# researchmm/MM-Diffusion

Hardware: AMD Instinct MI355X
Metric: denoising steps/sec (video+audio pair), 16x64x64 / 25600 (higher is better)
Workload: dtype bf16; 1 GPU; BASELINE configs[1]: Landscape base model (133.68M params), DDPM p_sample, timestep_respacing=250, per-GPU batch 4, 16x3x64x64 video + 1x25600 audio; global_batch=4, parallelism=batch-sharded x1, no in-loop collective, weights=key-seeded synthetic (mm_diffusion.synth), graph_replay=True, batch_lanes=2, finite=True, ranks_seen=1

## Files before the change

### include/mmd.h

```cpp
#ifndef MMD_H
#define MMD_H
#include <stdint.h>
#ifdef __cplusplus
extern "C" {
#endif

#define MMD_F32 0
#define MMD_BF16 1
#define MMD_OK 0
#define MMD_ERR_ARG (-1)
#define MMD_ERR_LAUNCH (-2)
#define MMD_ERR_UNSUPPORTED (-3)

int mmd_version(void);
const char* mmd_last_error(void);
int mmd_debug_install_crash_handler(void);

int mmd_graph_begin(void* stream);
int mmd_graph_end(void* stream, void** exec_out);
int mmd_graph_launch(void* exec, void* stream);
int mmd_graph_destroy(void* exec);
int mmd_stream_create(void** stream_out);
int mmd_stream_sync(void* stream);
int mmd_stream_destroy(void* stream);
int mmd_event_create(void** ev);
int mmd_event_record(void* ev, void* stream);
int mmd_stream_wait_event(void* stream, void* ev);
int mmd_event_elapsed_ms(void* ev_start, void* ev_stop, float* ms);
int mmd_event_destroy(void* ev);

int mmd_temb_fwd(const void* t, int t_kind, int N, int dim, const float* W0, const float* b0, const float* W2,
                 const float* b2, float* out_silu, float* out_raw, void* stream);

int mmd_linear_fwd(const float* x, const float* W, const float* b, float* y, int N, int K, int J, void* stream);

int64_t mmd_gn_workspace_bytes(int dtype, int C, int S, int Tn);
int mmd_gn_stats(int dtype, const void* x, int64_t ld, int C, int S, int Tn, int inner, int64_t outer_stride,
                 int64_t inner_stride, int64_t tstride, const float* gamma, const float* beta, const float* film,
                 int64_t film_ld, float eps, float* a_out, float* b_out, float* mr_out, void* workspace, void* stream);
int mmd_gn_finalize_stats(const float* rec, int64_t rec_ld, int C, int S, int Tn, const float* gamma, const float* beta,
                          const float* film, int64_t film_ld, float eps, float* a_out, float* b_out, float* mr_out, void* stream);
int mmd_gn_apply(int dtype, const void* x, int64_t ldx, void* y, int64_t ldy, int64_t rows, int C, int S, int Tn, int inner,
                 int64_t outer_stride, int64_t inner_stride, int64_t tstride, const float* a, const float* b, int act,
                 void* stream);
int mmd_add_rowbias(int dtype, void* x, int64_t ld, int64_t rows, int C, int64_t rows_per_sample, const float* e,
                    int64_t e_ld, void* stream);
int mmd_colsum_slices(int dtype, const void* dY, int64_t lddy, int S, int64_t Tn, int C, float* out, int64_t ldo, void* stream);

int mmd_conv_gemm(int dtype, const void* A, int64_t lda, const void* W, const float* bias, const void* R, int64_t ldr,
                  void* Y, int64_t ldy, int M, int Cout, int Cin, int ntaps, const int* taps, int D0, int D1, int D2, int tile,
                  void* stream);

int mmd_gn_conv1x1(int dtype, const void* A, int64_t lda, const float* gn_a, const float* gn_b, int act, int S,
                   int64_t rows_per_slice, const void* W, const float* bias, const void* R, int64_t ldr, void* Y, int64_t ldy,
                   int M, int Cout, int Cin, int tile, void* stream);

int mmd_gn_small(int dtype, const void* x, int64_t ldx, void* y, int64_t ldy, int C, int S, int Tn, int inner, int64_t outer_stride,
                 int64_t inner_stride, int64_t tstride, const float* gamma, const float* beta, float eps, int act, void* stream);

int mmd_gn_group(int dtype, const void* x, int64_t ldx, void* y, int64_t ldy, int C, int S, int Tn, int inner, int64_t outer_stride,
                 int64_t inner_stride, int64_t tstride, const float* gamma, const float* beta, const float* film, int64_t film_ld,
                 float eps, int act, float* a_out, float* b_out, float* mr_out, void* stream);

int mmd_zero(void* ptr, int64_t bytes, void* stream);

int mmd_conv_gemm_stats(int dtype, const void* A, int64_t lda, const void* W, const float* bias, const void* R, int64_t ldr,
                        void* Y, int64_t ldy, int M, int Cout, int Cin, int ntaps, const int* taps, int D0, int D1, int D2, int tile,
                        float* stats, int64_t stats_ld, void* stream);
int mmd_gn_conv1x1_stats(int dtype, const void* A, int64_t lda, const float* gn_a, const float* gn_b, int act, int S,
                         int64_t rows_per_slice, const void* W, const float* bias, const void* R, int64_t ldr, void* Y, int64_t ldy,
                         int M, int Cout, int Cin, int tile, float* stats, int64_t stats_ld, void* stream);

int mmd_gn_conv1x1_skip(int dtype, const void* h, int64_t ldh, const float* gn_a, const float* gn_b, int act, int S,
                        int64_t rows_per_slice, const void* W_out, const float* bias_out, const void* x, int64_t ldx, int K2,
                        const void* W_skip, const float* bias_skip, void* Y, int64_t ldy, int M, int Cout, int K1, float* stats,
                        int64_t stats_ld, void* stream);

int mmd_gn_conv_gemm(int dtype, const void* A, int64_t lda, const float* gn_a, const float* gn_b, int act, int S,
                     int64_t rows_per_slice, const void* W, const float* bias, const void* R, int64_t ldr, void* Y, int64_t ldy,
                     int M, int Cout, int Cin, int ntaps, const int* taps, int D0, int D1, int D2, int tile, void* stream);

int64_t mmd_vconv2d1d_weight_bytes(int Cin);
int mmd_vconv2d1d_pack(const void* Ws, const void* Wt, void* out, int Cin, int Cout, void* stream);
int mmd_vconv2d1d(const void* X, int64_t ldx, const float* gn_a, const float* gn_b, int act, int S, int64_t rows_per_slice,
                  const void* Wf, const float* bias_s, const float* bias_t, void* Y, int64_t ldy, int N, int F, int H, int W,
                  int Cin, int Cout, float* stats, int64_t stats_ld, void* stream);

int64_t mmd_tattn_weight_bytes(int C, int with_pre);
int mmd_tattn_pack(const void* Wpre, const void* Wqkv, const void* Wproj, void* out, int C, void* stream);
int mmd_tattn_block(const void* X, int64_t ldx, const void* A, int64_t lda, void* MID, int64_t ldm, const void* Wf,
                    const float* bias_pre, const float* bias_qkv, const float* bias_proj, const float* gamma, const float* beta,
                    float eps, void* Y, int64_t ldy, int N, int F, int HW, int C, int heads, float* stats, int64_t stats_ld,
                    void* stream);

int64_t mmd_tconv_weight_bytes(int Cin, int Cout);
int mmd_tconv_pack(const void* W, void* out, int Cin, int Cout, void* stream);
int mmd_tconv(const void* X, int64_t ldx, const void* Wf, const float* bias, void* Y, int64_t ldy, int N, int F, int HW, int Cin,
              int Cout, float* stats, int64_t stats_ld, void* stream);

int mmd_aconv(const void* X, int64_t ldx, const void* W, const float* bias, const float* ga, const float* gb, int act, void* Y, int64_t ldy,
              int M, int L, int Cin, int Cout, int dil, float* stats, int64_t stats_ld, void* stream);

int mmd_attn_fwd(int dtype, const void* Q, int64_t ldq, int q_off, const void* KV, int64_t ldkv, int k_off, int v_off, void* O,
                 int64_t ldo, int heads, int ch, int nb, int G, int64_t q_rows_per_batch, int q_per_group,
                 int64_t k_rows_per_batch, int k_per_group, int win, const int* shift_dev, int impl, void* stream);
int mmd_attn_small_fwd(int dtype, const void* QKV, int64_t ld, void* O, int64_t ldo, int C, int heads, int S, int Tn, int inner,
                       int64_t outer_stride, int64_t inner_stride, int64_t tstride, void* stream);

int mmd_resample(int dtype, const void* x, int64_t ldx, void* y, int64_t ldy, int C, int NF, int H, int W, int fh, int fw,
                 int mode, float scale, void* stream);
int mmd_resample_stats(const void* x, int64_t ldx, void* y, int64_t ldy, int C, int NF, int H, int W, int fh, int fw, int mode,
                       float* stats, int64_t stats_ld, void* stream);
int mmd_copy2d(const void* x, int64_t ldx_bytes, void* y, int64_t ldy_bytes, int64_t rows, int64_t row_bytes, void* stream);

int mmd_stem_conv(int dtype, const float* x, const float* w, const float* bias, void* y, int64_t ldy, int N, int F, int Cin,
                  int H, int W, int Cout, int ntaps, const int* taps, void* stream);
int mmd_head_conv(int dtype, const void* x, int64_t ldx, const float* w, const float* bias, float* y, int N, int F, int Cin,
                  int H, int W, int Co, int ntaps, const int* taps, void* stream);
int64_t mmd_head_gemm_weight_bytes(int Cin);
int64_t mmd_head_gemm_workspace_bytes(int64_t M, int ntaps, int Co);
int mmd_head_gemm(const void* x, int64_t ldx, int64_t M, int Cin, const float* gn_a, const float* gn_b, int S, int64_t gn_rows, int act,
                  const void* wimg, float* P, int NO, void* stream);
int mmd_head_gather(const float* P, const float* bias, float* y, int N, int F, int H, int W, int Co, int ntaps, const int* taps,
                    void* stream);

int mmd_ddpm_update(const float* x, const float* model_out, const float* noise, float* out, float* x0_out, float* mean_out,
                    float* logvar_out, const float* tables, const int64_t* t, int T, int N, int F, int C, int HW, int flags,
                    void* stream);
int mmd_q_sample(const float* x0, const float* eps, float* out, const float* tab2, const int64_t* t, int T, int N,
// ... 116 lines not shown
```

### mm-diffusion_amd/build.py

```python
#!/usr/bin/env python3
import os
import subprocess
import sys

HERE = os.path.dirname(os.path.abspath(__file__))
SRC = os.path.join(HERE, "csrc")
OUT = os.path.join(HERE, "lib", "libmmd.so")
SOURCES = ["mmd_core.hip", "mmd_gemm.hip", "mmd_vconv.hip", "mmd_tattn.hip", "mmd_tconv.hip", "mmd_aconv.hip", "mmd_norm.hip", "mmd_attn.hip", "mmd_misc.hip", "mmd_edge.hip", "mmd_diffusion.hip", "mmd_bwd.hip", "mmd_attn_bwd.hip", "mmd_attn_bwd_mfma.hip"]
FLAGS = ["--offload-arch=gfx950", "-O3", "-std=c++17", "-fPIC", "-ffp-contract=fast", "-Wno-unused-result", "-Wno-inline-asm"]
FLAGS += os.environ.get("MMD_EXTRA_CXXFLAGS", "").split()
NO_PACKED_F32 = ["-Xclang", "-target-feature", "-Xclang", "-packed-fp32-ops"]
FLAGS += NO_PACKED_F32


def _stale():
    if not os.path.exists(OUT):
        return True
    t = os.path.getmtime(OUT)
    deps = [os.path.join(SRC, f) for f in os.listdir(SRC)] + [os.path.abspath(__file__)]
    return any(os.path.getmtime(d) > t for d in deps)


def _llvm_bin():
    cands = [os.environ.get("LLVM_BIN")]
    hipcc = os.environ.get("HIPCC", "/opt/rocm/bin/hipcc")
    try:
        out = subprocess.run([hipcc, "--print-prog-name=llvm-objdump"], stdout=subprocess.PIPE, stderr=subprocess.DEVNULL, timeout=60).stdout.decode().strip()
        if out and os.path.isabs(out):
            cands.append(os.path.dirname(out))
    except (OSError, subprocess.SubprocessError):
        pass
    cands += [os.path.join(os.path.dirname(os.path.dirname(os.path.realpath(hipcc))), "lib", "llvm", "bin"), "/opt/rocm/lib/llvm/bin"]
    for d in cands:
        if d and os.path.exists(os.path.join(d, "llvm-objdump")):
            return d
    raise RuntimeError("build check: llvm-objdump not found (looked in %s); set LLVM_BIN to the LLVM bin directory of the ROCm toolchain"
                       % ", ".join(str(d) for d in cands if d))


def _code_objects(path, td):
    lib = os.path.join(td, os.path.basename(path))
    os.symlink(os.path.abspath(path), lib)
    subprocess.check_call([os.path.join(_llvm_bin(), "llvm-objdump"), "--offloading", lib], cwd=td, stdout=subprocess.DEVNULL, stderr=subprocess.DEVNULL)
    cos = [f for f in os.listdir(td) if f.startswith(os.path.basename(path) + ".") and f.endswith("gfx950")]
    return [os.path.join(td, f) for f in sorted(cos, key=lambda f: (len(f), f))]


def _check_no_packed_f32(path):
    import re
    import tempfile
    llvm = _llvm_bin()
    with tempfile.TemporaryDirectory() as td:
        cos = _code_objects(path, td)
        if len(cos) < len(SOURCES) - 1:
            raise RuntimeError("build check: expected >= %d gfx950 code objects in %s, found %d" % (len(SOURCES) - 1, path, len(cos)))
        asm = ""
        for f in cos:
            asm += subprocess.run([os.path.join(llvm, "llvm-objdump"), "-d", "--mcpu=gfx950", f],
                                  stdout=subprocess.PIPE, stderr=subprocess.DEVNULL, check=True).stdout.decode(errors="replace")
    n_mfma = len(re.findall(r"\bv_mfma_", asm))
    bad = re.findall(r"\bv_pk_(?:add|mul|fma)_f32\b", asm)
# ... 56 lines not shown
```

### mm-diffusion_amd/mm_diffusion/_hip.py

```python
import ctypes as C
import gc
import os

import torch

_HERE = os.path.dirname(os.path.abspath(__file__))
LIB_PATH = os.environ.get("MMD_LIB") or os.path.join(os.path.dirname(_HERE), "lib", "libmmd.so")

F32, BF16 = 0, 1
_lib = None

i32, i64, f32, vp = C.c_int, C.c_int64, C.c_float, C.c_void_p


_PROTOS = {
    "mmd_version": (C.c_int, []),
    "mmd_last_error": (C.c_char_p, []),
    "mmd_debug_install_crash_handler": (i32, []),
    "mmd_graph_begin": (i32, [vp]),
    "mmd_graph_end": (i32, [vp, C.POINTER(vp)]),
    "mmd_graph_launch": (i32, [vp, vp]),
    "mmd_graph_destroy": (i32, [vp]),
    "mmd_stream_create": (i32, [C.POINTER(vp)]),
    "mmd_stream_sync": (i32, [vp]),
    "mmd_stream_destroy": (i32, [vp]),
    "mmd_event_create": (i32, [C.POINTER(vp)]),
    "mmd_event_record": (i32, [vp, vp]),
    "mmd_stream_wait_event": (i32, [vp, vp]),
    "mmd_event_elapsed_ms": (i32, [vp, vp, C.POINTER(f32)]),
    "mmd_event_destroy": (i32, [vp]),
    "mmd_temb_fwd": (i32, [vp, i32, i32, i32, vp, vp, vp, vp, vp, vp, vp]),
    "mmd_linear_fwd": (i32, [vp, vp, vp, vp, i32, i32, i32, vp]),
    "mmd_gn_workspace_bytes": (i64, [i32, i32, i32, i32]),
    "mmd_gn_stats": (i32, [i32, vp, i64, i32, i32, i32, i32, i64, i64, i64, vp, vp, vp, i64, f32, vp, vp, vp, vp, vp]),
    "mmd_gn_small": (i32, [i32, vp, i64, vp, i64, i32, i32, i32, i32, i64, i64, i64, vp, vp, f32, i32, vp]),
    "mmd_gn_group": (i32, [i32, vp, i64, vp, i64, i32, i32, i32, i32, i64, i64, i64, vp, vp, vp, i64, f32, i32, vp, vp, vp, vp]),
    "mmd_gn_apply": (i32, [i32, vp, i64, vp, i64, i64, i32, i32, i32, i32, i64, i64, i64, vp, vp, i32, vp]),
    "mmd_add_rowbias": (i32, [i32, vp, i64, i64, i32, i64, vp, i64, vp]),
    "mmd_colsum_slices": (i32, [i32, vp, i64, i32, i64, i32, vp, i64, vp]),
    "mmd_conv_gemm": (i32, [i32, vp, i64, vp, vp, vp, i64, vp, i64, i32, i32, i32, i32, C.POINTER(i32), i32, i32, i32, i32, vp]),
    "mmd_gn_conv1x1": (i32, [i32, vp, i64, vp, vp, i32, i32, i64, vp, vp, vp, i64, vp, i64, i32, i32, i32, i32, vp]),
    "mmd_conv_gemm_stats": (i32, [i32, vp, i64, vp, vp, vp, i64, vp, i64, i32, i32, i32, i32, C.POINTER(i32), i32, i32, i32, i32, vp, i64, vp]),
    "mmd_gn_conv1x1_stats": (i32, [i32, vp, i64, vp, vp, i32, i32, i64, vp, vp, vp, i64, vp, i64, i32, i32, i32, i32, vp, i64, vp]),
    "mmd_gn_conv1x1_skip": (i32, [i32, vp, i64, vp, vp, i32, i32, i64, vp, vp, vp, i64, i32, vp, vp, vp, i64, i32, i32, i32, vp, i64, vp]),
    "mmd_gn_conv_gemm": (i32, [i32, vp, i64, vp, vp, i32, i32, i64, vp, vp, vp, i64, vp, i64, i32, i32, i32, i32, C.POINTER(i32), i32, i32, i32, i32, vp]),
    "mmd_tconv_weight_bytes": (i64, [i32, i32]),
    "mmd_tconv_pack": (i32, [vp, vp, i32, i32, vp]),
    "mmd_tconv": (i32, [vp, i64, vp, vp, vp, i64, i32, i32, i32, i32, i32, vp, i64, vp]),
    "mmd_aconv": (i32, [vp, i64, vp, vp, vp, vp, i32, vp, i64, i32, i32, i32, i32, i32, vp, i64, vp]),
    "mmd_tattn_weight_bytes": (i64, [i32, i32]),
    "mmd_tattn_pack": (i32, [vp, vp, vp, vp, i32, vp]),
    "mmd_tattn_block": (i32, [vp, i64, vp, i64, vp, i64, vp, vp, vp, vp, vp, vp, f32, vp, i64, i32, i32, i32, i32, i32, vp, i64, vp]),
    "mmd_vconv2d1d_weight_bytes": (i64, [i32]),
    "mmd_vconv2d1d_pack": (i32, [vp, vp, vp, i32, i32, vp]),
    "mmd_vconv2d1d": (i32, [vp, i64, vp, vp, i32, i32, i64, vp, vp, vp, vp, i64, i32, i32, i32, i32, i32, i32, vp, i64, vp]),
    "mmd_zero": (i32, [vp, i64, vp]),
    "mmd_gn_finalize_stats": (i32, [vp, i64, i32, i32, i32, vp, vp, vp, i64, f32, vp, vp, vp, vp]),
    "mmd_attn_fwd": (i32, [i32, vp, i64, i32, vp, i64, i32, i32, vp, i64, i32, i32, i32, i32, i64, i32, i64, i32, i32, vp, i32, vp]),
    "mmd_attn_small_fwd": (i32, [i32, vp, i64, vp, i64, i32, i32, i32, i32, i32, i64, i64, i64, vp]),
    "mmd_resample": (i32, [i32, vp, i64, vp, i64, i32, i32, i32, i32, i32, i32, i32, f32, vp]),
    "mmd_resample_stats": (i32, [vp, i64, vp, i64, i32, i32, i32, i32, i32, i32, i32, vp, i64, vp]),
    "mmd_copy2d": (i32, [vp, i64, vp, i64, i64, i64, vp]),
    "mmd_stem_conv": (i32, [i32, vp, vp, vp, vp, i64, i32, i32, i32, i32, i32, i32, i32, C.POINTER(i32), vp]),
    "mmd_head_conv": (i32, [i32, vp, i64, vp, vp, vp, i32, i32, i32, i32, i32, i32, i32, C.POINTER(i32), vp]),
    "mmd_head_gemm_weight_bytes": (i64, [i32]),
    "mmd_head_gemm_workspace_bytes": (i64, [i64, i32, i32]),
    "mmd_head_gemm": (i32, [vp, i64, i64, i32, vp, vp, i32, i64, i32, vp, vp, i32, vp]),
    "mmd_head_gather": (i32, [vp, vp, vp, i32, i32, i32, i32, i32, i32, C.POINTER(i32), vp]),
    "mmd_ddpm_update": (i32, [vp, vp, vp, vp, vp, vp, vp, vp, vp, i32, i32, i32, i32, i32, i32, vp]),
    "mmd_loss_workspace_bytes": (i64, [i32]),
    "mmd_loss_terms": (i32, [vp, vp, vp, vp, vp, vp, i32, i32, i32, i32, i32, i32, f32, vp, vp, vp, vp]),
    "mmd_conv_wgrad": (i32, [i32, vp, i64, vp, i64, vp, vp, i32, i32, i32, i32, C.POINTER(i32), i32, i32, i32, i32, vp]),
    "mmd_gn_bwd": (i32, [i32, vp, i64, vp, i64, vp, i64, i64, i32, i32, i32, i32, i64, i64, i64, vp, vp, vp, vp, vp, vp, i64, i32, vp, vp, vp, i64, vp, vp]),
    "mmd_gn_bwd_ws0": (i32, [i32, vp, i64, vp, i64, vp, i64, i64, i32, i32, i32, i32, i64, i64, i64, vp, vp, vp, vp, vp, vp, i64, i32, vp, vp, vp, i64, vp, vp]),
    "mmd_attn_bwd": (i32, [i32, vp, i64, i32, vp, i64, i32, i32, vp, i64, vp, i64, vp, i64, i32, vp, i64, i32, i32, vp, vp, i32, i32, i32, i32,
                           i32, i64, i64, i64, i32, i32, i32, i64, i64, i64, i32, i32, i32, vp, vp]),
    "mmd_timestep_embedding": (i32, [vp, i32, i32, i32, vp, vp]),
    "mmd_attn_fwd_lse": (i32, [i32, vp, i64, i32, vp, i64, i32, i32, vp, i64, i32, i32, i32, i32, i64, i32, i64, i32, i32, vp, vp, vp]),
    "mmd_attn_bwd_mfma": (i32, [vp, i64, i32, vp, i64, i32, i32, vp, i64, vp, i64, vp, i64, i32, vp, i64, i32, i32, vp, vp, i32, i32, i32, i32,
                                i64, i32, i64, i32, i32, vp, vp]),
    "mmd_attn_small_bwd": (i32, [i32, vp, i64, vp, i64, vp, i64, i32, i32, i32, i32, i32, i64, i64, i64, vp]),
    "mmd_ddim_update": (i32, [vp, vp, vp, vp, vp, vp, vp, vp, i32, i32, i32, i32, i32, i32, f32, vp]),
    "mmd_lincomb_t": (i32, [vp, vp, vp, vp, vp, vp, vp, i32, i64, vp]),
    "mmd_lincomb": (i32, [vp, f32, vp, f32, vp, f32, vp, i64, vp]),
    "mmd_cast": (i32, [vp, i32, vp, i32, f32, i64, vp]),
    "mmd_ddpm_update_bwd": (i32, [vp, vp, vp, vp, vp, vp, vp, i32, i32, i64, i32, vp]),
    "mmd_abs_quantile": (i32, [vp, i32, i64, f32, vp, vp]),
    "mmd_clamp_scale": (i32, [vp, vp, f32, i32, i64, vp]),
    "mmd_dpm_err": (i32, [vp, vp, vp, f32, f32, i32, i64, vp, vp]),
    "mmd_bilinear_concat": (i32, [vp, vp, vp, i32, i32, i32, i32, i32, i32, vp]),
    "mmd_bilinear_concat_rows": (i32, [i32, vp, vp, vp, i32, i32, i32, i32, i32, i32, i32, vp]),
    "mmd_pack_conv_weights": (i32, [i32, vp, i32, i32, vp]),
    "mmd_pack_blocks": (i32, [i32, i32, i32]),
    "mmd_unpack_conv_grads": (i32, [vp, i32, i32, vp]),
    "mmd_loss_terms_bwd": (i32, [vp, vp, vp, vp, vp, vp, i32, i32, i32, i32, i32, i32, f32, vp, vp, vp, vp]),
    "mmd_silu": (i32, [i32, vp, vp, vp, i64, vp]),
    "mmd_dropout": (i32, [i32, vp, vp, f32, vp, i64, vp]),
# ... 199 lines not shown
```

### mm-diffusion_amd/mm_diffusion/engine.py

```python
import os
from types import SimpleNamespace

import torch

from . import _hip as H
from . import ops
from .ops import Geom


_EMB_ON_AUDIO_STREAM = ops._flag("MMD_EMB_AUX")
_POOL_NOREUSE = os.environ.get("MMD_POOL_NOREUSE") == "1"
_UP_LOWRES = ops._flag("MMD_UP_LOWRES")
_CROSS_SERIAL = ops._flag("MMD_CROSS_SERIAL")
_RESAMPLE_STATS = ops._flag("MMD_RESAMPLE_STATS")
_SKIP_FUSE = ops._flag("MMD_SKIP_FUSE")


class _Pool:

    def __init__(self, device):
        self.device = device
        self.free = []
        self.all = []

    def get(self, nbytes):
        nbytes = (int(nbytes) + 255) // 256 * 256
        best = None
        for i, raw in enumerate(self.free):
            sz = raw.numel()
            if sz >= nbytes and sz <= 2 * nbytes + 65536 and (best is None or sz < self.free[best].numel()):
                best = i
        if best is not None:
            return self.free.pop(best)
        raw = torch.empty(nbytes, dtype=torch.uint8, device=self.device)
        self.all.append(raw)
        return raw

    def put(self, raw):
        if not _POOL_NOREUSE:
            self.free.append(raw)

    def total_bytes(self):
        return sum(r.numel() for r in self.all)


class UNetEngine:
    def __init__(self, model, N, dtype, device):
        if not torch.cuda.is_available():
            raise H.MMDError("no HIP device visible: the MI355X path cannot run (no CPU fallback)")
        H.lib()
        self.model, self.N, self.dtype, self.device = model, N, dtype, torch.device(device)
        self.F, self.Cv_in, self.H0, self.W0 = model.video_size
        self.Ca_in, self.L0 = model.audio_size
        self.mc = model.model_channels
        self.params = {k: v for k, v in model.named_parameters()}
        for k, v in self.params.items():
            if v.device.type != "cuda":
                raise H.MMDError(f"parameter {k} is on {v.device}: move the model to the GPU first (model.to('cuda'))")
        self._sig = self._signature()
        self.pools = [_Pool(self.device), _Pool(self.device)]
        mode = os.environ.get("MMD_GN_EPILOGUE", "1")
        self.rec_enabled = mode == "2" or (mode != "0" and dtype == torch.bfloat16)
        self._recs = {}
        self._gn_small = ops._flag("MMD_GN_SMALL")
        self._vconv_fused = self._tattn_fused = self._tconv = self._aconv = dtype == torch.bfloat16
        self._deferred = []
        H.reap()
        self._aux, self._side = H.Stream(self.device), H.Stream(self.device)
# ... 99 lines not shown
        return self._packed("edge", key, lambda: ops.pack_edge_weight(self.params[key].detach()))

    def _temporal(self, Hh):
        if ops.HALO_CANDIDATE:
            return dict(taps=ops.TAPS_TEMPORAL_D1, dims=(self.N, self.F, Hh * Hh))
        return dict(taps=ops.TAPS_TEMPORAL, dims=(self.F, Hh * Hh, 1))

    def _gn(self, x, prefix, geom, act, film=None, out=None):
        C = x.shape[1]
        if film is None and self._gn_small and ops.gn_small_ok(x, geom):
            y = self._alloc(x.shape[0], C) if out is None else out
            return ops.gn_small(x, self._f32(prefix + ".GroupNorm.weight"), self._f32(prefix + ".GroupNorm.bias"), geom, act=act, out=y)
        if ops.gn_group_ok(x, geom) and self._rec_ready(x, geom) is None:
            y = self._alloc(x.shape[0], C) if out is None else out
            return ops.gn_group(x, self._f32(prefix + ".GroupNorm.weight"), self._f32(prefix + ".GroupNorm.bias"), geom, film=film, out=y, act=act)
        a, b = self._gn_affine(x, prefix, geom, film)
        y = self._alloc(x.shape[0], C) if out is None else out
        ops.gn_apply(x, a, b, geom, act=act, out=y)
        self._release(a, b)
        return y

    def _gn_affine(self, x, prefix, geom, film):
        C = x.shape[1]
        a = self._alloc(geom.S, C, torch.float32)
        b = self._alloc(geom.S, C, torch.float32)
        gamma, beta = self._f32(prefix + ".GroupNorm.weight"), self._f32(prefix + ".GroupNorm.bias")
        rec = self._rec_ready(x, geom)
        if rec is not None:
            ops.gn_finalize_stats(rec, gamma, beta, geom, film=film, a=a, b=b)
        elif ops.gn_group_ok(x, geom):
            ops.gn_group(x, gamma, beta, geom, film=film, a=a, b=b)
        else:
            ws = self._alloc(ops.gn_workspace_bytes(x, geom) // 8, 1, torch.float64)
            ops.gn_stats(x, gamma, beta, geom, film=film, a=a, b=b, ws=ws)
            self._release(ws)
        return a, b

    def _gn_pw(self, x, gn_prefix, geom, act, wkey, bkey, film=None, residual=None, out=None):
        C = x.shape[1]
        Cout = self.params[wkey].shape[0]
        will_emit = True if (out is not None and self._rec_slice(out)[0] is not None) else None
        if not ops.gn_fusable(geom, C, Cout, x, will_emit, act):
            n1 = self._gn(x, gn_prefix, geom, act, film=film)
            y = self._pw(n1, wkey, bkey, residual=residual, out=out)
            self._release(n1)
            return y
        a, b = self._gn_affine(x, gn_prefix, geom, film)
        y = self._alloc(x.shape[0], Cout) if out is None else out
        ops.gn_conv1x1(x, a, b, geom, act, self._gemm_w(wkey), self._f32(bkey), residual=residual, out=y, **self._stats_kw(y))
        self._release(a, b)
        return y

    def _res_tail(self, s, h, xs, geom, film, make_out):
        if s.cin != s.cout and _SKIP_FUSE and ops.skip_fusable(h, xs, s.cout, geom):
            dest = make_out()
            will_emit = True if self._rec_slice(dest)[0] is not None else None
            if ops.skip_fusable(h, xs, s.cout, geom, will_emit, dest):
                a, b = self._gn_affine(h, s.out_norm, geom, film)
                (wo, bo), (wk, bk) = self._wb(s.out_conv), self._wb(s.skip)
                ops.gn_conv1x1_skip(h, a, b, geom, True, self._gemm_w(wo), self._f32(bo), xs, self._gemm_w(wk), self._f32(bk), out=dest,
                                    stats=self._stats_for(dest))
                self._release(a, b)
                return dest
            sk = self._pw(xs, *self._wb(s.skip))
        else:
            sk = self._pw(xs, *self._wb(s.skip)) if s.cin != s.cout else xs
            dest = make_out()
        self._gn_pw(h, s.out_norm, geom, True, *self._wb(s.out_conv), film=film, residual=sk, out=dest)
        if sk is not xs:
            self._release(sk)
        return dest

    def _pw(self, x, wkey, bkey, residual=None, out=None):
        y = self._alloc(x.shape[0], self.params[wkey].shape[0]) if out is None else out
        return ops.conv_gemm(x, self._gemm_w(wkey), self._f32(bkey), residual=residual, out=y, **self._stats_kw(y))

    def _self_attn(self, x, prefix, kind, Hh, out, pre=None, no_proj=False):
        N, F, C = self.N, self.F, x.shape[1]
        heads = self.model.num_heads
        ch = C // heads
        rows = x.shape[0]
        if kind == "spatial":
            geom = Geom.spatial(N, F, Hh * Hh)
        elif kind == "temporal":
            geom = Geom.temporal(N, F, Hh * Hh)
        else:
            geom = Geom.per_sample(N, rows // N)
        if kind == "temporal" and self._tattn_fused and ops.tattn_fused_ok(x, heads, N, F, Hh * Hh):
            pk = None
            if pre is not None:
                att, sp = pre
                mid = self._alloc(rows, C)
                pk = (att, self._f32(sp + ".proj_out.bias"), mid)
            wf = self._packed("tattn_pre" if pre is not None else "tattn", prefix, lambda: ops.tattn_pack(
                self._gemm_w(prefix + ".qkv.weight"), self._gemm_w(prefix + ".proj_out.weight"),
                wpre=self._gemm_w(pre[1] + ".proj_out.weight") if pre is not None else None))
            ops.tattn_block(x, wf, self._f32(prefix + ".qkv.bias"), self._f32(prefix + ".proj_out.bias"),
                            self._f32(prefix + ".norm.GroupNorm.weight"), self._f32(prefix + ".norm.GroupNorm.bias"), heads, N, F, Hh * Hh,
                            out=out, stats=self._stats_for(out, perm_unit=rows // N), pre=pk)
            if pk is not None:
                self._release(pk[2])
            return out
        qkv = self._gn_pw(x, prefix + ".norm", geom, False, prefix + ".qkv.weight", prefix + ".qkv.bias")
        att = self._alloc(rows, C)
        if kind == "temporal":
            if F > 32:
                raise H.MMDError(f"temporal attention over {F} frames: the short-sequence kernel handles <= 32")
            ops.attn_small(qkv, att, C, heads, geom)
        else:
            T = geom.Tn
            G = F if kind == "spatial" else 1
            ops.attn(qkv, qkv, att, heads, ch, N, G, G * T, T, G * T, T, 1)
        self._release(qkv)
        if no_proj:
            return att
# ... 395 lines not shown
```

### mm-diffusion_amd/mm_diffusion/ops.py

```python
import contextlib
import os

import torch

from . import _hip as H

GN_EPS = 1e-5

_recorder = None
_keep = None


class recording:
    def __init__(self, plan, keep=None):
        self.plan, self.keep = plan, keep

    def __enter__(self):
        global _recorder, _keep
        self._prev, _recorder = (_recorder, _keep), self.plan
        _keep = self.keep
        return self.plan

    def __exit__(self, *a):
        global _recorder, _keep
# ... 440 lines not shown
        raise H.MMDError("gn_conv1x1: the row-strip kernel is switched off (MMD_GEMM_STRIP) and the tiled loader cannot take this launch")
    if tile == 0:
        tile = _pick_tile((es, M, Cin, 1, Cout, residual is not None, True),
                          lambda t: H.call("mmd_gn_conv1x1", *base, t, H.stream_handle()), M, Cout,
                          candidates=(128,) if stats is not None else (64, 128), out=out, scratch=(x, residual, a, b))
    meta = _conv_meta("gn_conv1x1", x, Cout, 1, tile, residual)
    if stats is not None:
        _dispatch("mmd_gn_conv1x1_stats", *base, tile, *_stats_args(stats, M, Cout), meta=meta)
    else:
        _dispatch("mmd_gn_conv1x1", *base, tile, meta=meta)
    return out


_STRIP_K128_RF1 = os.environ.get("MMD_STRIP_K128_RF1", "1") != "0"


def skip_fusable(h, x, cout, geom: Geom, stats=None, out=None):
    if h.dtype != torch.bfloat16 or x.dtype != torch.bfloat16 or h.dim() != 2 or x.dim() != 2 or h.shape[0] != x.shape[0]:
        return False
    M, K1 = h.shape
    if K1 != 128 or x.shape[1] not in (256, 384) or cout % 32 or cout > 2048 or not _STRIP_K128_RF1:
        return False
    if not (geom.covers(M) and geom.Tn >= 16384) or (stats is not None and M % 64):
        return False
    if not strip_tile_pinned(h, cout, stats=stats, geom=geom) or not gn_fusable(geom, K1, cout, h, stats, act=True):
        return False
    ts = (h, x) + (() if out is None else (out,))
    if any(t.stride(1) != 1 or t.stride(0) % 8 or t.data_ptr() % 16 for t in ts):
        return False
    return M * (cout if out is None else out.stride(0)) * 2 < 0xffffffff


def gn_conv1x1_skip(h, a, b, geom: Geom, act, w, bias, x, w_skip, bias_skip, out=None, stats=None):
    _chk2d(h)
    _chk2d(x)
    M, K1 = h.shape
    K2 = x.shape[1]
    Cout = w.shape[0]
    _chk_conv_w("gn_conv1x1_skip", h, w, 1)
    _chk_conv_w("gn_conv1x1_skip", x, w_skip, 1)
    if x.shape[0] != M or w_skip.shape[0] != Cout:
        raise H.MMDError(f"gn_conv1x1_skip: h {tuple(h.shape)} / x {tuple(x.shape)} / skip weight {tuple(w_skip.shape)} do not match")
    out = alloc(M, Cout, dtype=h.dtype, device=h.device) if out is None else out
    _chk2d(out)
    es = h.element_size()
    meta = (f"gn_conv1x1_skip<{'bf16' if es == 2 else 'f32'},strip>[M={M},K={K1}+{K2},N={Cout}]", 2 * M * (K1 + K2) * Cout,
            es * (M * (K1 + K2) + M * Cout + Cout * (K1 + K2)) + 8 * Cout)
    _dispatch("mmd_gn_conv1x1_skip", H.dt_of(h), h.data_ptr(), h.stride(0), a.data_ptr(), b.data_ptr(), 1 if act else 0, geom.S, geom.Tn,
              w.data_ptr(), H.ptr(bias), x.data_ptr(), x.stride(0), K2, w_skip.data_ptr(), H.ptr(bias_skip), out.data_ptr(), out.stride(0),
              M, Cout, K1, *_stats_args(stats, M, Cout), meta=meta)
    return out


_HALO_GN = _flag("MMD_HALO_GN")


def halo_gn_ok(x, taps, dims, geom: Geom):
    return _HALO_GN and halo_tile_pinned(x, taps, dims) and geom.covers(x.shape[0]) and geom.Tn % (dims[1] * dims[2]) == 0


def gn_conv_gemm(x, a, b, geom: Geom, act, w, bias, taps, dims, residual=None, out=None, tile=0):
    _chk2d(x)
    M, Cin = x.shape
    Cout = w.shape[0]
    _chk_conv_w("gn_conv_gemm", x, w, len(taps))
    if not (halo_tile_ok(x, taps, dims) and len(taps) == 9 and x.dtype == torch.bfloat16 and geom.covers(M)
            and geom.Tn % (dims[1] * dims[2]) == 0):
        raise H.MMDError("gn_conv_gemm: needs a bf16 3x3 conv tile 130 accepts and contiguous slices of whole frames")
    out = alloc(M, Cout, dtype=x.dtype, device=x.device) if out is None else out
    _chk2d(out)
    arr, nt = H.taps_array(taps)
    tile = tile or halo_tile_code(x, taps, dims)
    _dispatch("mmd_gn_conv_gemm", H.dt_of(x), x.data_ptr(), x.stride(0), a.data_ptr(), b.data_ptr(), 1 if act else 0, geom.S, geom.Tn,
              w.data_ptr(), H.ptr(bias), H.ptr(residual), 0 if residual is None else residual.stride(0), out.data_ptr(), out.stride(0),
              M, Cout, Cin, nt, arr, int(dims[0]), int(dims[1]), int(dims[2]), tile,
              meta=_conv_meta("gn_conv_gemm", x, Cout, nt, tile, residual))
    return out


_VCONV_FUSED = _flag("MMD_VCONV_FUSED")


def vconv_shape_ok(x, Cout, N, F, Hh, Ww):
    return (x.dtype == torch.bfloat16 and F == 16 and Cout == 128 and x.shape[1] % 32 == 0 and Hh % 4 == 0 and Ww % 4 == 0
            and x.shape[0] == N * F * Hh * Ww and (16 * Hh * Ww * x.stride(0) + x.shape[1]) * 2 < 2 ** 31)


def _ranges_overlap(x, y):
    x0, y0 = x.data_ptr(), y.data_ptr()
    x1 = x0 + ((x.shape[0] - 1) * x.stride(0) + x.shape[1]) * x.element_size()
    y1 = y0 + ((y.shape[0] - 1) * y.stride(0) + y.shape[1]) * y.element_size()
    return not (x1 <= y0 or y1 <= x0)


def vconv_fused_ok(x, Cout, N, F, Hh, Ww, out=None):
    return _VCONV_FUSED and vconv_shape_ok(x, Cout, N, F, Hh, Ww) and (out is None or not _ranges_overlap(x, out))


def vconv_pack(ws, wt):
    H.require_cuda(ws, wt)
    Cout, Cin = ws.shape[0], ws.shape[1] // 9
    if ws.dtype != torch.bfloat16 or wt.dtype != torch.bfloat16 or tuple(wt.shape) != (Cout, 3 * Cout) or not ws.is_contiguous() or not wt.is_contiguous():
        raise H.MMDError(f"vconv_pack: expected contiguous bf16 [Cout, 9 Cin] / [Cout, 3 Cout], got {tuple(ws.shape)} / {tuple(wt.shape)}")
    out = torch.empty(H.lib().mmd_vconv2d1d_weight_bytes(Cin) // 2, dtype=torch.bfloat16, device=ws.device)
    H.call("mmd_vconv2d1d_pack", ws.data_ptr(), wt.data_ptr(), out.data_ptr(), Cin, Cout, H.stream_handle())
    return out
# ... 676 lines not shown
```

Measured before the change: 365.6 pair-steps/s.

## Add fused residual-tail kernel combining skip projection, out-conv and GN stats

Adds a new HIP kernel, res_tail, for channel-changing residual blocks where the existing strip-fused path does not apply. In one pass it computes the 1x1 skip projection of x and the GN-affine+SiLU 1x1 out-conv of h, adds biases and the residual, writes bf16 output and per-64-row group-norm statistics. It replaces a separate skip GEMM and a residual-add GEMM, so the intermediate skip tensor is never written or read back. Weights stream into LDS through a double-buffered ring of direct global-to-LDS loads, and blocks are remapped across XCDs. The path sits behind the MMD_TAIL_STREAM flag and shape heuristics, and it adds new code with detailed layout and stats-folding logic that could be wrong.

```diff
diff --git a/include/mmd.h b/include/mmd.h
--- a/include/mmd.h
+++ b/include/mmd.h
@@ -75,6 +75,10 @@
                         int64_t rows_per_slice, const void* W_out, const float* bias_out, const void* x, int64_t ldx, int K2,
                         const void* W_skip, const float* bias_skip, void* Y, int64_t ldy, int M, int Cout, int K1, float* stats,
                         int64_t stats_ld, void* stream);
+
+int mmd_res_tail(const void* h, int64_t ldh, const float* ga, const float* gb, int act, const void* W, const float* bias, const void* x,
+                 int64_t ldx, const void* W2, const float* bias2, void* Y, int64_t ldy, int M, int L, int K1, int K2, int Cout,
+                 float* stats, int64_t stats_ld, void* stream);
 
 int mmd_gn_conv_gemm(int dtype, const void* A, int64_t lda, const float* gn_a, const float* gn_b, int act, int S,
                      int64_t rows_per_slice, const void* W, const float* bias, const void* R, int64_t ldr, void* Y, int64_t ldy,
diff --git a/mm-diffusion_amd/build.py b/mm-diffusion_amd/build.py
--- a/mm-diffusion_amd/build.py
+++ b/mm-diffusion_amd/build.py
@@ -6,7 +6,7 @@
 HERE = os.path.dirname(os.path.abspath(__file__))
 SRC = os.path.join(HERE, "csrc")
 OUT = os.path.join(HERE, "lib", "libmmd.so")
-SOURCES = ["mmd_core.hip", "mmd_gemm.hip", "mmd_vconv.hip", "mmd_tattn.hip", "mmd_tconv.hip", "mmd_aconv.hip", "mmd_norm.hip", "mmd_attn.hip", "mmd_misc.hip", "mmd_edge.hip", "mmd_diffusion.hip", "mmd_bwd.hip", "mmd_attn_bwd.hip", "mmd_attn_bwd_mfma.hip"]
+SOURCES = ["mmd_core.hip", "mmd_gemm.hip", "mmd_vconv.hip", "mmd_tattn.hip", "mmd_tconv.hip", "mmd_aconv.hip", "mmd_rtail.hip", "mmd_norm.hip", "mmd_attn.hip", "mmd_misc.hip", "mmd_edge.hip", "mmd_diffusion.hip", "mmd_bwd.hip", "mmd_attn_bwd.hip", "mmd_attn_bwd_mfma.hip"]
 FLAGS = ["--offload-arch=gfx950", "-O3", "-std=c++17", "-fPIC", "-ffp-contract=fast", "-Wno-unused-result", "-Wno-inline-asm"]
 FLAGS += os.environ.get("MMD_EXTRA_CXXFLAGS", "").split()
 NO_PACKED_F32 = ["-Xclang", "-target-feature", "-Xclang", "-packed-fp32-ops"]
diff --git a/mm-diffusion_amd/csrc/mmd_rtail.hip b/mm-diffusion_amd/csrc/mmd_rtail.hip
--- /dev/null
+++ b/mm-diffusion_amd/csrc/mmd_rtail.hip
@@ -0,0 +1,284 @@
+#include "mmd_common.h"
+#include <type_traits>
+
+struct RTailParams {
+  const char* H; int64_t ldh;
+  const char* X; int64_t ldx;
+  const char* W;
+  const char* W2;
+  const float* bias; const float* bias2;
+  const float* ga; const float* gb;
+  char* Y; int64_t ldy;
+  float* stats; int64_t stats_ld;
+  int M, L, K1, K2, Cout, act;
+  int pair;
+};
+
+template <int CSUB, bool GN, int KB>
+__global__ __launch_bounds__(256, 2) void rtail_kernel(const RTailParams p, const int nsplit) {
+  constexpr int CS = 32 * CSUB;
+  constexpr int PLANE_B = CS * 128;
+  constexpr int STAGE_B = KB * PLANE_B;
+  constexpr int NCG = 4 * KB;
+  constexpr int GP = CS / 32;
+  static_assert(2 * STAGE_B >= 2 * CSUB * 2 * 64 * 16, "the two-fragment fold parks two waves' stored values in the weight ring");
+  extern __shared__ __attribute__((aligned(16))) char smem[];
+  char* sW = smem;
+  float* sBias = (float*)(smem + 2 * STAGE_B);
+  float* sBias2 = sBias + CS;
+  float* sRec = sBias2 + CS;
+  float* sAB = sRec + 4 * CSUB * 2 * 2 * 2 * 2;
+
+  const int tid = threadIdx.x, lane = tid & 63;
+  const int wave = __builtin_amdgcn_readfirstlane(tid >> 6);
+  const int half = lane >> 5, l31 = lane & 31;
+  const int nwg = gridDim.x;
+  int wgid;
+  {
+    const int bid = blockIdx.x, q = nwg >> 3, r = nwg & 7, xcd = bid & 7;
+    wgid = (xcd < r ? xcd * (q + 1) : r * (q + 1) + (xcd - r) * q) + (bid >> 3);
+  }
+  const int sp = wgid % nsplit, mt = wgid / nsplit;
+  const int cbase = sp * CS, m0 = mt * 128;
+  const int n2 = p.K2 / (64 * KB), nsteps = n2 + p.K1 / (64 * KB);
+
+  typedef const __attribute__((address_space(1))) void* gptr_t;
+  typedef __attribute__((address_space(3))) void* lptr_t;
+  const int lrow = lane >> 3, pc = lane & 7;
+  const char *w_ptr[GP], *w2_ptr[GP];
+#pragma unroll
+  for (int ih = 0; ih < GP; ++ih) {
+    const int row = 8 * (ih * 4 + wave) + lrow;
+    const int logical = pc ^ ((row >> 1) & 7);
+    w_ptr[ih] = p.W + ((int64_t)(cbase + row) * p.K1 + logical * 8) * 2;
+    w2_ptr[ih] = p.W2 + ((int64_t)(cbase + row) * p.K2 + logical * 8) * 2;
+  }
+  auto issue_w = [&](int stage, int s) {
+#pragma unroll
+    for (int pl = 0; pl < KB; ++pl)
+#pragma unroll
+      for (int ih = 0; ih < GP; ++ih) {
+        const char* src = s < n2 ? w2_ptr[ih] + (int64_t)(s * KB + pl) * 128 : w_ptr[ih] + (int64_t)((s - n2) * KB + pl) * 128;
+        __builtin_amdgcn_global_load_lds((gptr_t)src, (lptr_t)(sW + stage * STAGE_B + pl * PLANE_B + (ih * 4 + wave) * 1024), 16, 0, 0);
+      }
+  };
+  const int row = m0 + wave * 32 + l31;
+  const bool rok = row < p.M;
+  const int rowc = rok ? row : p.M - 1;
+  const int s0 = m0 / p.L;
+  const int gsel = min(rowc / p.L - s0, 1) * 2 * p.K1;
+  auto load_act = [&](int s, u32x4 (&x)[NCG]) {
+    const bool second = s < n2;
+    const char* base = second ? p.X : p.H;
+    const int64_t ld = second ? p.ldx : p.ldh;
+    const int ck = second ? s : s - n2;
+    const char* ap = base + ((int64_t)rowc * ld + ck * (64 * KB) + half * 8) * 2;
+#pragma unroll
+    for (int cg = 0; cg < NCG; ++cg) x[cg] = *(const u32x4*)(ap + cg * 32);
+  };
+
+  issue_w(0, 0);
+  u32x4 xc[NCG], xn[NCG];
+  load_act(0, xc);
+  if (tid < CS) {
+    sBias[tid] = p.bias ? p.bias[cbase + tid] : 0.f;
+    sBias2[tid] = p.bias2 ? p.bias2[cbase + tid] : 0.f;
+  }
+  if constexpr (GN) {
+    const int nS = p.M / p.L;
+    for (int i = tid; i < 4 * p.K1; i += 256) {
+      const int sl = i / (2 * p.K1), ab = (i / p.K1) & 1, c = i % p.K1;
+      const int sidx = min(s0 + sl, nS - 1);
+      sAB[i] = (ab ? p.gb : p.ga)[(int64_t)sidx * p.K1 + c];
+    }
+  }
+  f32x16 acc[CSUB], acc2[CSUB];
+#pragma unroll
+  for (int a = 0; a < CSUB; ++a)
+#pragma unroll
+    for (int r = 0; r < 16; ++r) acc[a][r] = acc2[a][r] = 0.f;
+  asm volatile("s_waitcnt vmcnt(0)" ::: "memory");
+  __syncthreads();
+
+  const int xsw = (l31 >> 1) & 7;
+  auto step = [&](int s, auto norm, f32x16 (&ac)[CSUB]) __attribute__((always_inline)) {
+    const int st = s & 1;
+    if (s + 1 < nsteps) {
+      issue_w(st ^ 1, s + 1);
+      load_act(s + 1, xn);
+    }
+    if constexpr (decltype(norm)::value) {
+      const int ck = s - n2;
+#pragma unroll
+      for (int cg = 0; cg < NCG; ++cg) {
+        float x[8];
+        Elt<__bf16>::unpack(xc[cg], x);
+        const float* ap = sAB + gsel + ck * (64 * KB) + cg * 16 + half * 8;
+        const float* bp = ap + p.K1;
+#pragma unroll
+        for (int e = 0; e < 8; e += 4) {
+          const f32x4 av = *(const f32x4*)(ap + e), bv = *(const f32x4*)(bp + e);
+#pragma unroll
+          for (int k = 0; k < 4; ++k) {
+            const float y = x[e + k] * av[k] + bv[k];
+            x[e + k] = p.act ? silu_f(y) : y;
+          }
+        }
+        xc[cg] = Elt<__bf16>::pack(x);
+      }
+    }
+    const char* bW = sW + st * STAGE_B + l31 * 128;
+#pragma unroll
+    for (int cg = 0; cg < NCG; ++cg)
+#pragma unroll
+      for (int a = 0; a < CSUB; ++a) {
+        const u32x4 fw = *(const u32x4*)(bW + (cg >> 2) * PLANE_B + a * 32 * 128 + (((2 * (cg & 3) + half) ^ xsw) * 16));
+        ac[a] = __builtin_amdgcn_mfma_f32_32x32x16_bf16(__builtin_bit_cast(bf16x8, fw), __builtin_bit_cast(bf16x8, xc[cg]), ac[a], 0, 0, 0);
+      }
+    asm volatile("s_waitcnt vmcnt(0)" ::: "memory");
+    __syncthreads();
+#pragma unroll
+    for (int cg = 0; cg < NCG; ++cg) xc[cg] = xn[cg];
+  };
+  int s = 0;
+  for (; s < n2; ++s) step(s, std::false_type{}, acc2);
+  for (; s < nsteps; ++s) step(s, std::integral_constant<bool, GN>{}, acc);
+
+  const bool wave_ok = (int64_t)m0 + wave * 32 < p.M;
+  const int64_t rec = ((int64_t)m0 + wave * 32) / 64;
+  u32x4* sPk = (u32x4*)sW;
+  float srec[CSUB][2][4];
+#pragma unroll
+  for (int a = 0; a < CSUB; ++a)
+#pragma unroll
+    for (int j2 = 0; j2 < 2; ++j2) {
+      const int cb = a * 32 + 16 * j2 + 8 * half;
+      const f32x4 b0 = *(const f32x4*)(sBias + cb), b1 = *(const f32x4*)(sBias + cb + 4);
+      const f32x4 c0 = *(const f32x4*)(sBias2 + cb), c1 = *(const f32x4*)(sBias2 + cb + 4);
+      float v[8], sk[8], rf[8];
+#pragma unroll
+      for (int j = 0; j < 4; ++j) {
+        const auto sw = __builtin_amdgcn_permlane32_swap(__float_as_uint(acc[a][8 * j2 + j]), __float_as_uint(acc[a][8 * j2 + 4 + j]), false, false);
+        v[j] = __uint_as_float(sw[0]);
+        v[4 + j] = __uint_as_float(sw[1]);
+      }
+#pragma unroll
+      for (int j = 0; j < 4; ++j) { v[j] += b0[j]; v[4 + j] += b1[j]; }
+#pragma unroll
+      for (int j = 0; j < 4; ++j) {
+        const auto sw = __builtin_amdgcn_permlane32_swap(__float_as_uint(acc2[a][8 * j2 + j]), __float_as_uint(acc2[a][8 * j2 + 4 + j]), false, false);
+        sk[j] = __uint_as_float(sw[0]) + c0[j];
+        sk[4 + j] = __uint_as_float(sw[1]) + c1[j];
+      }
+      Elt<__bf16>::unpack(Elt<__bf16>::pack(sk), rf);
+#pragma unroll
+      for (int j = 0; j < 8; ++j) v[j] += rf[j];
+      const u32x4 pk = Elt<__bf16>::pack(v);
+      if (rok) *(u32x4*)(p.Y + ((int64_t)rowc * p.ldy + cbase + cb) * 2) = pk;
+      if (p.stats) {
+        if (p.pair && (wave & 1)) {
+          sPk[((wave >> 1) * (CSUB * 2) + a * 2 + j2) * 64 + lane] = pk;
+          continue;
+        }
+        float u[4] = {0.f, 0.f, 0.f, 0.f};
+        Elt<__bf16>::unpack(pk, rf);
+#pragma unroll
+        for (int j = 0; j < 4; ++j) {
+          u[0] += rf[j];
+          u[1] += rf[4 + j];
+          u[2] += rf[j] * rf[j];
+          u[3] += rf[4 + j] * rf[4 + j];
+        }
+        if (p.pair) {
+#pragma unroll
+          for (int k = 0; k < 4; ++k) srec[a][j2][k] = u[k];
+          continue;
+        }
+        const float t0 = halfwave_total(u[0]), t1 = halfwave_total(u[1]), t2 = halfwave_total(u[2]), t3 = halfwave_total(u[3]);
+        const float msum = (l31 & 1) ? t1 : t0, msq = (l31 & 1) ? t3 : t2;
+        srec[a][j2][0] = msum;
+        srec[a][j2][1] = msq;
+        if ((wave & 1) && (l31 >> 1) == 8) {
+          float* d = sRec + (((wave * CSUB + a) * 2 + j2) * 2 + half) * 4 + (l31 & 1) * 2;
+          d[0] = msum;
+          d[1] = msq;
+        }
+      }
+    }
+  if (p.stats) {
+    __syncthreads();
+    if (wave_ok && (wave & 1) == 0) {
+#pragma unroll
+      for (int a = 0; a < CSUB; ++a)
+#pragma unroll
+        for (int j2 = 0; j2 < 2; ++j2) {
+          const int col = cbase + a * 32 + 16 * j2 + 8 * half;
+          float* d = p.stats + (rec * p.stats_ld + (col >> 2) + (l31 & 1)) * 2;
+          if (p.pair) {
+            float u[4], rf[8];
+#pragma unroll
+            for (int k = 0; k < 4; ++k) u[k] = srec[a][j2][k];
+            Elt<__bf16>::unpack(sPk[((wave >> 1) * (CSUB * 2) + a * 2 + j2) * 64 + lane], rf);
+#pragma unroll
+            for (int j = 0; j < 4; ++j) {
+              u[0] += rf[j];
+              u[1] += rf[4 + j];
+              u[2] += rf[j] * rf[j];
+              u[3] += rf[4 + j] * rf[4 + j];
+            }
+            const float t0 = halfwave_total(u[0]), t1 = halfwave_total(u[1]), t2 = halfwave_total(u[2]), t3 = halfwave_total(u[3]);
+            if ((l31 >> 1) == 8) {
+              d[0] = (l31 & 1) ? t1 : t0;
+              d[1] = (l31 & 1) ? t3 : t2;
+            }
+          } else if ((l31 >> 1) == 8) {
+            const float* o = sRec + ((((wave + 1) * CSUB + a) * 2 + j2) * 2 + half) * 4 + (l31 & 1) * 2;
+            d[0] = srec[a][j2][0] + o[0];
+            d[1] = srec[a][j2][1] + o[1];
+          }
+        }
+    }
+  }
+}
+
+template <int CSUB, bool GN, int KB>
+static int launch_rtail(const RTailParams& p, hipStream_t st) {
+  constexpr int CS = 32 * CSUB;
+  const int rowblocks = cdiv(p.M, 128), nsplit = p.Cout / CS;
+  constexpr size_t FIXED = 2 * (size_t)KB * CS * 128 + 2 * (size_t)CS * 4 + 4 * CSUB * 2 * 2 * 2 * 2 * 4;
+  const size_t lds = FIXED + (GN ? 4 * (size_t)p.K1 * 4 : 0);
+  const size_t lds_max = FIXED + 4 * (size_t)512 * 4;
+  return mmd_launch_cap<rtail_kernel<CSUB, GN, KB>>("res_tail", dim3(rowblocks * nsplit), dim3(256), lds, lds_max, st, p, nsplit);
+}
+
+template <bool GN>
+static int dispatch_rtail(RTailParams& p, hipStream_t st) {
+  p.pair = p.K1 == 256 || (p.K1 == 128 && (!GN || p.L < 16384));
+  if (p.Cout % 128 == 0 && (int64_t)cdiv(p.M, 128) * (p.Cout / 128) >= 192) return launch_rtail<4, GN, 1>(p, st);
+  if (p.K1 % 128 == 0 && p.K2 % 128 == 0) return launch_rtail<2, GN, 2>(p, st);
+  return launch_rtail<2, GN, 1>(p, st);
+}
+
+extern "C" int mmd_res_tail(const void* h, int64_t ldh, const float* ga, const float* gb, int act, const void* W, const float* bias,
+                            const void* x, int64_t ldx, const void* W2, const float* bias2, void* Y, int64_t ldy, int M, int L, int K1,
+                            int K2, int Cout, float* stats, int64_t stats_ld, void* stream) {
+  MMD_REQUIRE(h && x && W && W2 && Y, "res_tail: null pointer");
+  MMD_REQUIRE((ga == nullptr) == (gb == nullptr), "res_tail: the fused affine needs both ga and gb (or neither: h is already normalised)");
+  MMD_REQUIRE(M > 0 && L >= 128 && M % L == 0, "res_tail: M = %d rows must be whole samples of L = %d >= 128 rows", M, L);
+  MMD_REQUIRE(K1 == 128 || K1 == 256 || K1 == 384 || K1 == 512, "res_tail: K1 = %d must be 128, 256, 384 or 512", K1);
+  MMD_REQUIRE(K2 >= 64 && K2 % 64 == 0 && K2 <= 1024, "res_tail: K2 = %d must be a multiple of 64 up to 1024", K2);
+  MMD_REQUIRE(Cout > 0 && Cout % 64 == 0, "res_tail: Cout = %d must be a multiple of 64", Cout);
+  MMD_REQUIRE(ldh >= K1 && ldx >= K2 && ldy >= Cout && ldh % 8 == 0 && ldx % 8 == 0 && ldy % 8 == 0 &&
+                  ((uintptr_t)h | (uintptr_t)x | (uintptr_t)W | (uintptr_t)W2 | (uintptr_t)Y) % 16 == 0,
+              "res_tail: rows must be 16-byte aligned");
+  MMD_REQUIRE(!stats || (M % 64 == 0 && stats_ld >= Cout / 4 && (uintptr_t)stats % 8 == 0),
+              "res_tail: statistics need M %% 64 == 0 and a record row of >= Cout / 4 quads");
+  const char *y0 = (const char*)Y, *y1 = y0 + ((int64_t)(M - 1) * ldy + Cout) * 2;
+  const char *h0 = (const char*)h, *h1 = h0 + ((int64_t)(M - 1) * ldh + K1) * 2, *x0 = (const char*)x, *x1 = x0 + ((int64_t)(M - 1) * ldx + K2) * 2;
+  MMD_REQUIRE((h1 <= y0 || y1 <= h0) && (x1 <= y0 || y1 <= x0), "res_tail: h / x and Y overlap (the column ranges of a row block read rows the others write)");
+  RTailParams p;
+  p.H = h0; p.ldh = ldh; p.X = x0; p.ldx = ldx; p.W = (const char*)W; p.W2 = (const char*)W2; p.bias = bias; p.bias2 = bias2;
+  p.ga = ga; p.gb = gb; p.Y = (char*)Y; p.ldy = ldy; p.stats = stats; p.stats_ld = stats_ld;
+  p.M = M; p.L = L; p.K1 = K1; p.K2 = K2; p.Cout = Cout; p.act = act; p.pair = 0;
+  return ga ? dispatch_rtail<true>(p, (hipStream_t)stream) : dispatch_rtail<false>(p, (hipStream_t)stream);
+}
diff --git a/mm-diffusion_amd/mm_diffusion/_hip.py b/mm-diffusion_amd/mm_diffusion/_hip.py
--- a/mm-diffusion_amd/mm_diffusion/_hip.py
+++ b/mm-diffusion_amd/mm_diffusion/_hip.py
@@ -43,6 +43,7 @@
     "mmd_conv_gemm_stats": (i32, [i32, vp, i64, vp, vp, vp, i64, vp, i64, i32, i32, i32, i32, C.POINTER(i32), i32, i32, i32, i32, vp, i64, vp]),
     "mmd_gn_conv1x1_stats": (i32, [i32, vp, i64, vp, vp, i32, i32, i64, vp, vp, vp, i64, vp, i64, i32, i32, i32, i32, vp, i64, vp]),
     "mmd_gn_conv1x1_skip": (i32, [i32, vp, i64, vp, vp, i32, i32, i64, vp, vp, vp, i64, i32, vp, vp, vp, i64, i32, i32, i32, vp, i64, vp]),
+    "mmd_res_tail": (i32, [vp, i64, vp, vp, i32, vp, vp, vp, i64, vp, vp, vp, i64, i32, i32, i32, i32, i32, vp, i64, vp]),
     "mmd_gn_conv_gemm": (i32, [i32, vp, i64, vp, vp, i32, i32, i64, vp, vp, vp, i64, vp, i64, i32, i32, i32, i32, C.POINTER(i32), i32, i32, i32, i32, vp]),
     "mmd_tconv_weight_bytes": (i64, [i32, i32]),
     "mmd_tconv_pack": (i32, [vp, vp, i32, i32, vp]),
diff --git a/mm-diffusion_amd/mm_diffusion/engine.py b/mm-diffusion_amd/mm_diffusion/engine.py
--- a/mm-diffusion_amd/mm_diffusion/engine.py
+++ b/mm-diffusion_amd/mm_diffusion/engine.py
@@ -14,6 +14,7 @@
 _CROSS_SERIAL = ops._flag("MMD_CROSS_SERIAL")
 _RESAMPLE_STATS = ops._flag("MMD_RESAMPLE_STATS")
 _SKIP_FUSE = ops._flag("MMD_SKIP_FUSE")
+_TAIL_STREAM = ops._TAIL_STREAM
 
 
 class _Pool:
@@ -219,15 +220,30 @@
         return y
 
     def _res_tail(self, s, h, xs, geom, film, make_out):
-        if s.cin != s.cout and _SKIP_FUSE and ops.skip_fusable(h, xs, s.cout, geom):
+        changing = s.cin != s.cout
+        strip = changing and ops.skip_fusable(h, xs, s.cout, geom)
+        stream = changing and not strip and _TAIL_STREAM and ops.res_tail_ok(h, xs, s.cout, geom) and ops.res_tail_pays(h, xs)
+        if (strip and _SKIP_FUSE) or stream:
             dest = make_out()
             will_emit = True if self._rec_slice(dest)[0] is not None else None
-            if ops.skip_fusable(h, xs, s.cout, geom, will_emit, dest):
+            (wo, bo), (wk, bk) = self._wb(s.out_conv), self._wb(s.skip)
+            if strip and ops.skip_fusable(h, xs, s.cout, geom, will_emit, dest):
                 a, b = self._gn_affine(h, s.out_norm, geom, film)
-                (wo, bo), (wk, bk) = self._wb(s.out_conv), self._wb(s.skip)
                 ops.gn_conv1x1_skip(h, a, b, geom, True, self._gemm_w(wo), self._f32(bo), xs, self._gemm_w(wk), self._f32(bk), out=dest,
                                     stats=self._stats_for(dest))
                 self._release(a, b)
+                return dest
+            if stream and ops.res_tail_ok(h, xs, s.cout, geom, will_emit, dest):
+                if ops.res_tail_norm_fused(h, s.cout, geom, will_emit):
+                    a, b = self._gn_affine(h, s.out_norm, geom, film)
+                    ops.res_tail(h, a, b, geom, True, self._gemm_w(wo), self._f32(bo), xs, self._gemm_w(wk), self._f32(bk), out=dest,
+                                 stats=self._stats_for(dest))
+                    self._release(a, b)
+                else:
+                    n1 = self._gn(h, s.out_norm, geom, True, film=film)
+                    ops.res_tail(n1, None, None, geom, True, self._gemm_w(wo), self._f32(bo), xs, self._gemm_w(wk), self._f32(bk), out=dest,
+                                 stats=self._stats_for(dest))
+                    self._release(n1)
                 return dest
             sk = self._pw(xs, *self._wb(s.skip))
         else:
diff --git a/mm-diffusion_amd/mm_diffusion/ops.py b/mm-diffusion_amd/mm_diffusion/ops.py
--- a/mm-diffusion_amd/mm_diffusion/ops.py
+++ b/mm-diffusion_amd/mm_diffusion/ops.py
@@ -516,6 +516,66 @@
     return out
 
 
+_TAIL_STREAM = _flag("MMD_TAIL_STREAM")
+_TAIL_NORM = os.environ.get("MMD_TAIL_NORM", "")
+_TAIL_NORM_FUSED_K1 = (256, 384)
+
+
+def res_tail_ok(h, x, cout, geom: Geom, stats=None, out=None):
+    if h.dtype != torch.bfloat16 or x.dtype != torch.bfloat16 or h.dim() != 2 or x.dim() != 2 or h.shape[0] != x.shape[0]:
+        return False
+    M, K1 = h.shape
+    K2 = x.shape[1]
+    if K1 not in (128, 256, 384, 512) or K2 % 64 or not 64 <= K2 <= 1024 or cout % 64 or cout <= 0:
+        return False
+    if not (geom.covers(M) and geom.Tn >= 128) or (stats is not None and M % 64):
+        return False
+    if not strip_tile_pinned(h, cout, stats=stats):
+        return False
+    if K1 == 128 and geom.Tn >= 16384 and not _STRIP_K128_RF1:
+        return False
+    ts = (h, x) + (() if out is None else (out,))
+    if any(t.stride(1) != 1 or t.stride(0) % 8 or t.data_ptr() % 16 for t in ts):
+        return False
+    return out is None or not (_ranges_overlap(h, out) or _ranges_overlap(x, out))
+
+
+def res_tail_pays(h, x):
+    return h.shape[1] != 512 or x.shape[1] > 512
+
+
+def res_tail_norm_fused(h, cout, geom: Geom, stats=None):
+    K1 = h.shape[1]
+    if K1 == 128:
+        return strip_tile_pinned(h, cout, stats=stats, geom=geom) and gn_fusable(geom, K1, cout, h, stats, act=True)
+    if _TAIL_NORM in ("0", "1"):
+        return _TAIL_NORM == "1"
+    return K1 in _TAIL_NORM_FUSED_K1
+
+
+def res_tail(h, a, b, geom: Geom, act, w, bias, x, w_skip, bias_skip, out=None, stats=None):
+    _chk2d(h)
+    _chk2d(x)
+    M, K1 = h.shape
+    K2 = x.shape[1]
+    Cout = w.shape[0]
+    _chk_conv_w("res_tail", h, w, 1)
+    _chk_conv_w("res_tail", x, w_skip, 1)
+    if x.shape[0] != M or w_skip.shape[0] != Cout or h.dtype != torch.bfloat16 or not geom.covers(M) or (a is None) != (b is None):
+        raise H.MMDError(f"res_tail: h {tuple(h.shape)} {h.dtype} / x {tuple(x.shape)} / skip weight {tuple(w_skip.shape)} do not match, "
+                         "or the slices are not whole contiguous samples")
+    if a is not None and not all(tuple(t.shape) == (geom.S, K1) and t.dtype == torch.float32 and t.is_contiguous() for t in (a, b)):
+        raise H.MMDError(f"res_tail: the fused affine must be two contiguous fp32 [S, K1] tensors (got {tuple(a.shape)}, {tuple(b.shape)})")
+    out = alloc(M, Cout, dtype=h.dtype, device=h.device) if out is None else out
+    _chk2d(out)
+    meta = (f"res_tail<bf16,stream>[M={M},K={K1}+{K2},N={Cout}]", 2 * M * (K1 + K2) * Cout,
+            2 * (M * (K1 + K2) + M * Cout + Cout * (K1 + K2)) + 8 * Cout)
+    _dispatch("mmd_res_tail", h.data_ptr(), h.stride(0), H.ptr(a), H.ptr(b), 1 if act else 0, w.data_ptr(), H.ptr(bias), x.data_ptr(),
+              x.stride(0), w_skip.data_ptr(), H.ptr(bias_skip), out.data_ptr(), out.stride(0), M, geom.Tn, K1, K2, Cout,
+              *_stats_args(stats, M, Cout), meta=meta)
+    return out
+
+
 _HALO_GN = _flag("MMD_HALO_GN")
 
 
```

Result: faster. 373.9 pair-steps/s, median of 6 (+2.3%).
